# edouardlp/Mask-RCNN-CoreML

Hardware: AMD Instinct MI355X
Metric: images/sec (1024x1024, COCO-80) (higher is better)
Workload: dtype f32x3

## Files before the change

### mask-rcnn-coreml_amd/csrc/conv_dispatch.hip

```cpp
#include "conv_device.h"
#include "knobs.h"

namespace mrcnn {

void conv_mfma_launch(hipStream_t s, const ConvArgs& a, int mode, int bn, bool wide_waves);
void conv_pp_launch(hipStream_t s, const ConvArgs& a, int mode);
void conv_chain_launch(hipStream_t s, const ConvArgs& p, const ConvArgs& q, int parts, int n_cus, const void* p_stream, const void* q_stream);

static inline int conv_wdtype(const ConvDesc& d) { return d.wdtype < 0 ? d.dtype : d.wdtype; }
static inline bool conv_is_split(const ConvDesc& d) { return d.dtype == MRCNN_F32 && (conv_wdtype(d) == MRCNN_F16 || conv_wdtype(d) == MRCNN_F32X3); }
static inline int conv_split_parts(const ConvDesc& d) { return conv_wdtype(d) == MRCNN_F32X3 ? 3 : 2; }
static inline bool conv_is_f16(const ConvDesc& d) { return d.dtype == MRCNN_F16 && (d.wdtype < 0 || d.wdtype == MRCNN_F16) && !d.out_f32; }
static inline bool is_pointwise(const ConvDesc& d) { return d.KH == 1 && d.KW == 1 && d.stride == 1 && !d.padH && !d.padW; }
static inline bool is_3x3_same(const ConvDesc& d) { return d.KH == 3 && d.KW == 3 && d.stride == 1 && d.padH == 1 && d.padW == 1; }
static inline bool dense_in(const ConvDesc& d, int h, int w, int c) { return d.H == h && d.W == w && d.Cin == c && d.in_sW == c && d.in_sH == (long)w * c && d.in_sB == (long)h * w * c; }
static inline bool dense_out(const ConvDesc& d, int h, int w, int c) { return d.OH == h && d.OW == w && d.Cout == c && d.out_sP == c && d.out_sB == (long)h * w * c; }
static inline bool plain_epilogue(const ConvDesc& d, int act) { return !d.out2 && !d.deconv2 && !d.sel_partial && !d.head_w && d.res_shift == 0 && d.act == act && d.scale && d.shift; }
static inline bool fills_chip(long tiles, int n_cus) { return tiles * 8 >= (long)n_cus * 7; }

static thread_local ConvProfile* g_prof = nullptr;
void conv_set_profiler(ConvProfile* p) { g_prof = p; }
static thread_local int* g_range_flag = nullptr;
void conv_set_range_flag(int* device_flag) { g_range_flag = device_flag; }
void ConvProfile::reset()
// ... 43 lines not shown
}
static int prof_event(ConvProfile* p, hipStream_t s)
{
    if (p->used == (int)p->pool.size()) {
        hipEvent_t e;
        HIP_CHECK(hipEventCreate(&e));
        p->pool.push_back(e);
    }
    HIP_CHECK(hipEventRecord(p->pool[p->used], s));
    return p->used++;
}
struct ProfScope {
    ConvProfile* const prof = (g_prof && g_prof->active) ? g_prof : nullptr;
    const hipStream_t s;
    const int e0;
    explicit ProfScope(hipStream_t s_) : s(s_), e0(prof ? prof_event(prof, s_) : 0) {}
    explicit operator bool() const { return prof != nullptr; }
    void finish(ConvTileClass tile, double flops, int M, int N, int K, int group, double bytes) const
    {
        const int e1 = prof_event(prof, s);
        prof->pending.push_back({tile, flops, e0, e1, {M, N, K, tile}, group, bytes});
    }
};

int conv_n_tile(int Cout)
{
    if (Cout > 64) return 128;
    if (Cout > 32) return 64;
    return 32;
}

static int& g_min_blocks = knob("conv_min_blocks", nullptr, 448);
static int& g_min_blocks_split = knob("conv_min_blocks_split", nullptr, 256, "conv_min_blocks");
static inline int min_blocks_for(bool split_mode) { return split_mode ? g_min_blocks_split : g_min_blocks; }
static int& g_direct = knob("conv_direct", "MRCNN_DIRECT", 3);
static int& g_stem = knob("conv_stem", "MRCNN_STEM", 1);
static int& g_tail_dbg = knob("conv_tail_dbg", "MRCNN_TAIL_DBG", 0);
static int& g_tail = knob("conv_tail", "MRCNN_TAIL", 0);
static int& g_bneck = knob("conv_bneck", "MRCNN_BNECK", 1);
static int& g_bneck_stage = knob("conv_bneck_stage", "MRCNN_BNECK_STAGE", 0);
static int& g_c3h = knob("conv_c3h", "MRCNN_C3H", 1);
int conv_c3h_mode() { return g_c3h; }
bool conv_bneck_enabled() { return g_bneck != 0; }
static int& g_scfuse = knob("conv_scfuse", "MRCNN_SCFUSE", 1);
static int& g_sel_wave = knob("mask_sel_wave", "MRCNN_SEL_WAVE", 1);
int conv_sel_part_cols() { return g_sel_wave ? 64 : 128; }
static int& g_kchunk = knob("conv_kchunk", "MRCNN_KCHUNK", 1);
static int& g_ksplit = knob("conv_ksplit", "MRCNN_KSPLIT", 1);
static int& g_ksplit_below = knob("conv_ksplit_below", "MRCNN_KSPLIT_BELOW", 256);
static int& g_halo = knob("conv_halo", "MRCNN_HALO", 1);
bool conv_halo_enabled() { return g_halo != 0; }
static int& g_chain = knob("conv_chain", "MRCNN_CHAIN", 1);
static int& g_chain4 = knob("conv_chain4", "MRCNN_CHAIN4", 1);
static int& g_tn4 = knob("conv_tn4", nullptr, -1);

static int& g_pp = knob("conv_pp", "MRCNN_PP", 1);
static int& g_pp_min_tiles = knob("conv_pp_min_tiles", "MRCNN_PP_MIN_TILES", 512);
static int& g_pp_min_kt = knob("conv_pp_min_kt", "MRCNN_PP_MIN_KT", 16);
static int& g_pp_dbg = knob("conv_pp_dbg", "MRCNN_PP_DBG", 0);
static int& g_pp_min_fill = knob("conv_pp_min_fill", "MRCNN_PP_MIN_FILL", 85);
static int& g_pp_split = knob("conv_pp_split", "MRCNN_PP_SPLIT", 0);

static void conv_fill_args(const ConvDesc& d, ConvArgs& a)
{
    const bool half = d.dtype == MRCNN_F16;
    a.in = d.in; a.wgt = d.wgt; a.scale = d.scale; a.shift = d.shift; a.res = d.res; a.out = d.out; a.out2 = d.out2;
    a.in_sB = d.in_sB; a.in_sH = d.in_sH; a.in_sW = d.in_sW;
    a.res_sB = d.res_sB; a.res_sH = d.res_sH; a.res_sW = d.res_sW;
    a.out_sB = d.out_sB; a.out_sP = d.out_sP; a.out_sH = d.out_sH; a.out_sW = d.out_sW;
    a.out2_sB = d.out2_sB; a.out2_sP = d.out2_sP;
    a.B = d.B; a.H = d.H; a.W = d.W; a.Cin = d.Cin; a.KH = d.KH; a.KW = d.KW; a.stride = d.stride; a.padH = d.padH; a.padW = d.padW;
    a.OH = d.OH; a.OW = d.OW; a.Cout = d.Cout;
    a.ncols = d.deconv2 ? 4 * d.Cout : d.Cout;
    a.Ktot = d.KH * d.KW * d.Cin;
    const long M = (long)d.B * d.OH * d.OW;
    MRCNN_REQUIRE(M > 0 && M < (1L << 31) - 256, MRCNN_ERR_SHAPE, "conv: M out of range");
    a.M = (int)M;
    a.res_shift = d.res_shift; a.act = d.act; a.n_split = d.n_split; a.deconv2 = d.deconv2;
    a.out_f32 = (!half || d.out_f32) ? 1 : 0;
    a.range_flag = g_range_flag;
    a.dbg = g_pp_dbg;
    a.sel_w = d.sel_w; a.sel_cid = d.sel_cid; a.sel_partial = d.sel_partial;
    a.kchunks = 1; a.ksplit = 1; a.ks_scratch = nullptr; a.ks_count = nullptr;
    a.sel_part_cols = 128;
    a.sc_in = nullptr; a.sc_wgt = nullptr; a.sc_scale = nullptr; a.sc_shift = nullptr;
    a.sc_in_sB = a.sc_in_sH = a.sc_in_sW = 0; a.sc_H = a.sc_W = a.sc_Cin = 0; a.sc_stride = 1;
}

int conv_k_chunks(const ConvDesc& d)
{
    if (!g_kchunk || !conv_is_split(d) || d.KH != 1 || d.KW != 1 || d.Cin < 2048 || d.Cin % 32 != 0 || d.head_w) return 1;
    int n = d.Cin >= 8192 ? 8 : 4;
    while ((d.Cin / 32) % n) n >>= 1;
    return n;
}

static constexpr size_t KS_BYTES = 64u << 20;
static constexpr int KS_TILES = 8192;
static thread_local ConvScratch* g_scratch = nullptr;
void conv_set_scratch(ConvScratch* c) { g_scratch = c; }
size_t ConvScratch::ks_bytes() { return KS_BYTES; }
void ConvScratch::alloc()
{
    ks_buf.alloc(KS_BYTES);
    ks_cnt.alloc(KS_TILES * sizeof(unsigned));
    HIP_CHECK(hipMemset(ks_cnt.p, 0, KS_TILES * sizeof(unsigned)));
// ... 122 lines not shown
    if (pp_bn) conv_pp_launch(s, a, half ? 0 : parts);
    else conv_mfma_launch(s, a, half ? 0 : (split ? parts : 1), bn, wide_waves);
    if (prof) {
        const double k = (d.algo_k > 0 ? d.algo_k : a.Ktot) + (fuse ? sc->Cin : 0);
        const ConvTileClass tile = halo ? TILE_HALO : pp_bn == 256 ? TILE_PP_256x256 : (wide_waves ? TILE_128x128_4WAVE : (bn == 128 ? TILE_128x128 : (bn == 64 ? TILE_128x64 : TILE_128x32)));
        prof.finish(tile, 2.0 * (double)a.M * (double)a.ncols * k, a.M, a.ncols, a.Ktot, d.group, conv_algorithmic_bytes(d, fuse ? sc : nullptr));
    }
    HIP_CHECK(hipGetLastError());
}

bool conv_stem_enabled() { return g_stem != 0; }
bool conv_stem_eligible(const ConvDesc& d)
{
    const bool half = conv_is_f16(d);
    const int pxc = half ? 8 : 4;
    return (conv_is_split(d) || half) && d.KH == 7 && d.KW == 1 && d.Cin == 8 * pxc && d.stride == 2 && d.padH == 0 && d.padW == 0 && d.Cout == 64 && d.Npad == 64 &&
           d.act == ACT_RELU && !d.res && !d.out2 && !d.deconv2 && d.in_sW == pxc && d.in_sH == (long)d.W * pxc && d.in_sB == (long)d.H * d.W * pxc &&
           d.OH == (d.H - 7) / 2 + 1 && d.OW == (d.W - 7) / 2 + 1;
}

void conv_stem_forward(hipStream_t s, const ConvDesc& d, void* pooled, int PH, int PW)
{
    MRCNN_REQUIRE(conv_stem_eligible(d) && pooled && PH == (d.OH + 1) / 2 && PW == (d.OW + 1) / 2, MRCNN_ERR_INVALID, "conv_stem_forward: not the stem layer");
    const int n_cus = device_cu_count();
    const ProfScope prof(s);
    conv_stem_launch(s, d.in, d.B, d.H, d.W, d.wgt, d.scale, d.shift, d.OH, d.OW, pooled, PH, PW,
                     d.dtype == MRCNN_F16 ? 1 : conv_split_parts(d), g_range_flag, n_cus, g_stem != 2);
    if (prof) {
        const long M = (long)d.B * d.OH * d.OW;
        const double k = d.algo_k > 0 ? d.algo_k : d.KH * d.KW * d.Cin;
        const double by = (double)d.B * d.H * d.W * 16.0 + 64.0 * k * 2.0 + (double)d.B * PH * PW * 64.0 * (d.dtype == MRCNN_F16 ? 2.0 : 4.0);
        prof.finish(TILE_128x64, 2.0 * (double)M * 64.0 * k, (int)M, 64, d.KH * d.KW * d.Cin, d.group, by);
    }
}

bool conv_tail_fusable(const ConvDesc& d3, const ConvDesc& d1)
{
    if (!conv_is_split(d3) || !conv_is_split(d1) || conv_wdtype(d3) != conv_wdtype(d1)) return false;
    if (!d3.wgt_halo || !d1.wgt_halo || !conv_halo_eligible(d3) || d3.head_w || !conv_halo_tail_geometry_ok(d3.H, d3.W)) return false;
    if (d3.Npad != 256 || d3.act != ACT_RELU) return false;
    if (!conv_halo_tail_packable(d1.KH, d1.KW, d1.Cin, d1.Npad) || d1.Cout != 1024 || !is_pointwise(d1)) return false;
    if (d1.deconv2 || d1.out2 || d1.sel_partial || d1.act == ACT_SIGMOID || d1.res_shift || d1.head_w) return false;
    if (d1.in != d3.out || d1.B != d3.B || d1.OH != d3.OH || d1.OW != d3.OW) return false;
    if (!dense_out(d3, d3.OH, d3.OW, 256) || !dense_in(d1, d3.OH, d3.OW, 256)) return false;
    return true;
}

bool conv_chain_fusable(const ConvDesc& dP, const ConvDesc& dQ, const ConvDesc* sc)
{
    if (!conv_is_split(dP) || !conv_is_split(dQ) || conv_wdtype(dP) != conv_wdtype(dQ)) return false;
    const int C = dQ.Cout, H = dP.OH, W = dP.OW;
    if (!(C == 64 || C == 128 || C == 256) || dQ.Npad != C || dP.Cin != C || dP.Cout != 4 * C || dP.Npad != 4 * C) return false;
    if (!is_pointwise(dP) || !is_pointwise(dQ) || dP.B != dQ.B) return false;
    if (!plain_epilogue(dP, ACT_RELU) || !plain_epilogue(dQ, ACT_RELU) || dQ.res) return false;
    if (!dense_in(dP, H, W, C) || !dense_out(dP, H, W, 4 * C) || dQ.in != dP.out || !dense_in(dQ, H, W, 4 * C) || !dense_out(dQ, H, W, C)) return false;
    if (conv_k_chunks(dP) != 1 || conv_k_chunks(dQ) != 1) return false;
    auto al = [](const void* p) { return (reinterpret_cast<uintptr_t>(p) & 15) == 0; };
    if (!al(dP.in) || !al(dP.out) || !al(dQ.out) || !al(dP.wgt) || !al(dQ.wgt) || !al(dP.scale) || !al(dP.shift) || !al(dQ.scale) || !al(dQ.shift)) return false;
    if (C == 256 && (sc || !dP.wgt_stream || !dQ.wgt_stream || !al(dP.wgt_stream) || !al(dQ.wgt_stream))) return false;
    if (sc) {
        if (!g_scfuse || !conv_shortcut_fusable(dP, *sc) || conv_k_chunks(*sc) != 1 || !sc->scale || !sc->shift) return false;
        if (C == 64 && sc->Cin != 64) return false;
        if (!al(sc->in) || !al(sc->wgt) || !al(sc->scale) || !al(sc->shift) || sc->in_sW % 4 || sc->in_sH % 4 || sc->in_sB % 4 || sc->Npad != 4 * C) return false;
    } else {
        if (!dP.res || !al(dP.res) || dP.res_sW != 4 * C || dP.res_sH != (long)W * 4 * C || dP.res_sB != (long)H * W * 4 * C) return false;
    }
    return true;
}

void conv_forward_chain(hipStream_t s, const ConvDesc& dP, const ConvDesc& dQ, const ConvDesc* sc)
{
    const long tiles = ((long)dP.B * dP.OH * dP.OW + 127) / 128;
    const bool sc_rides = g_chain >= 3 ? sc != nullptr && conv_chain_fusable(dP, dQ, sc) : conv_shortcut_rides(dP, sc);
    const int n_cus = device_cu_count();
    const bool c4 = dQ.Cout == 256;
    const int g = c4 ? g_chain4 : g_chain;
    bool chain = g && g_direct >= 2 && !(c4 && sc) && conv_chain_fusable(dP, dQ, sc_rides ? sc : nullptr) && (g >= 2 || ((c4 || dQ.Cout == 64) && fills_chip(tiles, n_cus)));
#ifndef MRCNN_CONV_ABLATE
    if (g_pp_dbg) chain = false;
#endif
    if (!chain) {
        conv_forward(s, dP, sc);
        conv_forward(s, dQ);
        return;
    }
    if (sc && !sc_rides) { conv_forward(s, *sc); sc = nullptr; }
    ConvDesc d = dP;
    if (sc) { d.res = nullptr; d.res_sB = d.res_sH = d.res_sW = 0; }
    ConvArgs aP, aQ;
    conv_fill_args(d, aP);
    conv_fill_args(dQ, aQ);
    if (sc) {
        aP.sc_in = sc->in; aP.sc_wgt = sc->wgt; aP.sc_scale = sc->scale; aP.sc_shift = sc->shift;
        aP.sc_in_sB = sc->in_sB; aP.sc_in_sH = sc->in_sH; aP.sc_in_sW = sc->in_sW;
        aP.sc_H = sc->H; aP.sc_W = sc->W; aP.sc_Cin = sc->Cin; aP.sc_stride = sc->stride;
    }
    const ProfScope prof(s);
    conv_chain_launch(s, aP, aQ, conv_split_parts(dP), n_cus, dP.wgt_stream, dQ.wgt_stream);
    if (prof) {
        const double fl = 2.0 * (double)aP.M * ((double)aP.ncols * (aP.Ktot + (sc ? sc->Cin : 0)) + (double)aQ.ncols * aQ.Ktot);
        prof.finish(sc ? TILE_128x128_4WAVE : TILE_128x128, fl, aP.M, aP.ncols, aP.Ktot, dP.group,
                    conv_algorithmic_bytes(d, sc) + conv_algorithmic_bytes(dQ) - (double)aP.M * dQ.Cin * 4.0);
    }
    HIP_CHECK(hipGetLastError());
}

void conv_forward_tail(hipStream_t s, const ConvDesc& d3, const ConvDesc& d1, const ConvDesc* sc, const ConvDesc* q)
{
    const int n_cus = device_cu_count();
    const long tiles = ((long)d3.B * d3.OH * d3.OW + 127) / 128;
    ConvArgs a3, a1;
    bool fuse = g_tail && g_halo && g_scratch && conv_tail_fusable(d3, d1) && fills_chip(tiles, n_cus);
    if (sc && fuse) { conv_forward(s, *sc); sc = nullptr; }
    if (fuse) {
        conv_fill_args(d3, a3);
        conv_fill_args(d1, a1);
        a3.vec_ok = conv_vec_ok(d3, a3);
        a1.vec_ok = conv_vec_ok(d1, a1);
        a3.tiles_m = a1.tiles_m = 0; a3.tiles_n = a1.tiles_n = 0; a3.direct = a1.direct = 1;
        a1.dbg = g_tail_dbg;
        fuse = a3.vec_ok && a1.vec_ok && a3.dbg == 0;
    }
    if (!fuse) {
        conv_forward(s, d3);
        if (q) conv_forward_chain(s, d1, *q, sc);
        else conv_forward(s, d1, sc);
        return;
    }
    const ProfScope prof(s);
    (void)conv_halo_forward(s, a3, d3, conv_split_parts(d3), n_cus, &a1, d1.wgt_halo);
    if (prof) {
        const double fl = 2.0 * (double)a3.M * ((double)a3.ncols * a3.Ktot + (double)a1.ncols * a1.Ktot);
        ConvDesc d3n = d3; d3n.sel_partial = (float*)1;
        prof.finish(TILE_HALO_TAIL, fl, a3.M, a1.ncols, a3.Ktot + a1.Ktot, d3.group, conv_algorithmic_bytes(d3n) + conv_algorithmic_bytes(d1) - (double)a3.M * d1.Cin * 4.0);
    }
    HIP_CHECK(hipGetLastError());
    if (q) conv_forward(s, *q);
}

bool conv_bneck_fusable(const ConvDesc& da, const ConvDesc& db, const ConvDesc& dc)
{
    if (!conv_is_f16(da) || !conv_is_f16(db) || !conv_is_f16(dc)) return false;
    const int C = da.Cout, H = da.H, W = da.W;
    if (!(C == 64 || C == 128 || C == 256) || !bneck_geometry_ok(C, H, W)) return false;
    if (!plain_epilogue(da, ACT_RELU) || !plain_epilogue(db, ACT_RELU) || !plain_epilogue(dc, ACT_RELU) || da.res || db.res) return false;
    if (!is_pointwise(da) || !dense_in(da, H, W, 4 * C) || !dense_out(da, H, W, C)) return false;
    if (!is_3x3_same(db) || db.in != da.out || !dense_in(db, H, W, C) || !dense_out(db, H, W, C)) return false;
    if (!is_pointwise(dc) || dc.in != db.out || !dense_in(dc, H, W, C) || !dense_out(dc, H, W, 4 * C)) return false;
    if (dc.res != da.in || dc.res_sW != 4 * C || dc.res_sH != (long)W * 4 * C || dc.res_sB != (long)H * W * 4 * C) return false;
    if (dc.out == da.in) return false;
    if (da.B != db.B || da.B != dc.B) return false;
// ... 88 lines not shown
```

### mask-rcnn-coreml_amd/csrc/conv_pack.h

```cpp
#pragma once
#include <stddef.h>
#include <vector>

namespace mrcnn {

template <class Src>
std::vector<float> pack_filter_rows(int O, int I, int KH, int KW, int Npad, Src&& src)
{
    std::vector<float> w((size_t)Npad * KH * KW * I, 0.f);
    for (int o = 0; o < O; ++o)
        for (int y = 0; y < KH; ++y)
            for (int x = 0; x < KW; ++x)
                for (int i = 0; i < I; ++i) w[(((size_t)o * KH + y) * KW + x) * I + i] = src(o, y, x, i);
    return w;
}

inline int deconv2_row(int dy, int dx, int co, int O) { return (dy * 2 + dx) * O + co; }
template <class Src>
std::vector<float> pack_deconv2_rows(int I, int O, int Npad, Src&& src)
{
    std::vector<float> w((size_t)Npad * I, 0.f);
    for (int dy = 0; dy < 2; ++dy)
        for (int dx = 0; dx < 2; ++dx)
            for (int o = 0; o < O; ++o)
                for (int i = 0; i < I; ++i) w[(size_t)deconv2_row(dy, dx, o, O) * I + i] = src(dy, dx, o, i);
    return w;
}

inline bool chain_stream_wanted(int KH, int KW, int I, int O) { return KH == 1 && KW == 1 && ((I == 256 && O == 1024) || (I == 1024 && O == 256)); }
inline size_t chain_stream_pos_p(int C, int n, int k)
{
    const int r = n & 63;
    return (size_t)(n >> 6) * 64 * C + ((size_t)(k >> 5) * 64 + r) * 32 + ((((k >> 3) & 3) ^ ((r >> 2) & 3)) << 3) + (k & 7);
}
inline size_t chain_stream_pos_q(int C, int n, int k)
{
    return (size_t)(k >> 6) * 64 * C + ((size_t)((k >> 5) & 1) * C + n) * 32 + ((((k >> 3) & 3) ^ ((n >> 2) & 3)) << 3) + (k & 7);
}
template <class T>
std::vector<T> pack_chain_stream(const T* w, int C, bool q)
{
    static_assert(sizeof(T) == 2, "fp16 filters");
    const int rows = q ? C : 4 * C, K = q ? 4 * C : C;
    std::vector<T> img((size_t)rows * K);
    for (int n = 0; n < rows; ++n)
        for (int k = 0; k < K; ++k) img[q ? chain_stream_pos_q(C, n, k) : chain_stream_pos_p(C, n, k)] = w[(size_t)n * K + k];
    return img;
}

}
```

### mask-rcnn-coreml_amd/csrc/engine_weights.hip

```cpp
#include "engine_internal.h"
#include "conv_pack.h"

#include <math.h>
#include <string.h>

#include <fstream>

namespace mrcnn {

float half_to_float(uint16_t h)
{
    const uint32_t sign = (uint32_t)(h & 0x8000u) << 16;
    uint32_t exp = (h >> 10) & 0x1Fu, man = h & 0x3FFu, f;
    if (exp == 0) {
        if (man == 0) f = sign;
        else {
            exp = 113;
            while ((man & 0x400u) == 0) { man <<= 1; --exp; }
            man &= 0x3FFu;
            f = sign | (exp << 23) | (man << 13);
        }
    } else if (exp == 31) f = sign | 0x7F800000u | (man << 13);
    else f = sign | ((exp + 112) << 23) | (man << 13);
    float r;
// ... 146 lines not shown
    shift.assign(Npad, 0.f);
    if (bn.empty()) {
        for (int o = 0; o < Cout; ++o) { scale[o] = 1.f; shift[o] = bias[o]; }
        return;
    }
    const std::vector<float> g = f.floats(bn + "/gamma"), be = f.floats(bn + "/beta"), mu = f.floats(bn + "/mean"),
                             var = f.floats(bn + "/variance");
    const float eps = (float)f.get_double("bn_eps", 1e-3);
    for (int o = 0; o < Cout; ++o) {
        const float sc = g[o] / sqrtf(var[o] + eps);
        scale[o] = sc;
        shift[o] = (bias[o] - mu[o]) * sc + be[o];
    }
}

static PackedConv new_pack(int mode, int Cin, int Cout, int KH, int KW)
{
    PackedConv pc;
    pc.dtype = mode_act(mode); pc.wdtype = mode_wgt(mode);
    pc.Cin = Cin; pc.Cout = Cout; pc.KH = KH; pc.KW = KW;
    const int bn_tile = conv_n_tile(Cout);
    pc.Npad = (Cout + bn_tile - 1) / bn_tile * bn_tile;
    return pc;
}
static void finish_pack(PackedConv& pc, const std::vector<float>& w, const std::vector<float>& sc, const std::vector<float>& sh)
{
    upload_w(pc.wgt, w, pc.wdtype, pc.wdtype != pc.dtype, "MRCNN_F32S / MRCNN_F32X3");
    upload(pc.scale, sc);
    upload(pc.shift, sh);
    pc.h_scale = sc; pc.h_shift = sh;
}

PackedConv pack_conv_oihw(const MrcwFile& f, const std::string& conv, const std::string& bn, int dtype)
{
    const MrcwTensor& t = f.tensor(conv + "/kernel");
    MRCNN_REQUIRE(t.dims.size() == 4, MRCNN_ERR_IO, "%s/kernel is not 4-D", conv.c_str());
    const int O = t.dims[0], I = t.dims[1], KH = t.dims[2], KW = t.dims[3];
    const std::vector<float> k = f.floats(conv + "/kernel");
    PackedConv pc = new_pack(dtype, I, O, KH, KW);
    const std::vector<float> w = pack_filter_rows(O, I, KH, KW, pc.Npad, [&](int o, int y, int x, int i) { return k[(((size_t)o * I + i) * KH + y) * KW + x]; });
    std::vector<float> sc, sh;
    fold_bn(f, conv, bn, O, pc.Npad, sc, sh);
    finish_pack(pc, w, sc, sh);
    if (pc.wdtype != pc.dtype && conv_halo_packable(KH, KW, I, pc.Npad)) {
        conv_halo_pack(nullptr, pc.wgt.p, pc.Npad, I, pc.wgt_halo);
        HIP_CHECK(hipStreamSynchronize(nullptr));
    } else if (pc.wdtype != pc.dtype && conv_halo_tail_packable(KH, KW, I, pc.Npad) && O == pc.Npad) {
        conv_halo_pack(nullptr, pc.wgt.p, pc.Npad, I, pc.wgt_halo, 1);
        HIP_CHECK(hipStreamSynchronize(nullptr));
    }
    if (pc.wdtype != pc.dtype && pc.dtype == MRCNN_F32 && O == pc.Npad && chain_stream_wanted(KH, KW, I, O) && conv.find("_branch2") != std::string::npos) {
        std::vector<uint16_t> hw(w.size());
        for (size_t i = 0; i < w.size(); ++i) hw[i] = float_to_half(w[i]);
        const std::vector<uint16_t> img = pack_chain_stream(hw.data(), 256, I == 1024);
        pc.wgt_stream.alloc(img.size() * 2);
        HIP_CHECK(hipMemcpy(pc.wgt_stream.p, img.data(), img.size() * 2, hipMemcpyHostToDevice));
    }
    if (pc.dtype == MRCNN_F16 && pc.wdtype == MRCNN_F16 && conv3x3h_packable(KH, KW, I, O, pc.Npad)) {
        conv3x3h_pack(nullptr, pc.wgt.p, O, I, pc.wgt_c3h);
        HIP_CHECK(hipStreamSynchronize(nullptr));
    }
    if (pc.dtype == MRCNN_F16 && pc.wdtype == MRCNN_F16 && O == pc.Npad && bneck_frag_wanted(KH, KW, I, O)) {
        bneck_pack_frag(nullptr, pc.wgt.p, O, KH * KW * I, pc.wgt_frag);
        HIP_CHECK(hipStreamSynchronize(nullptr));
    }
    return pc;
}

PackedConv pack_conv1(const MrcwFile& f, int dtype)
{
    const MrcwTensor& t = f.tensor("conv1/kernel");
    MRCNN_REQUIRE(t.dims.size() == 4 && t.dims[1] == 3 && t.dims[2] == 7 && t.dims[3] == 7, MRCNN_ERR_IO, "conv1/kernel must be [O,3,7,7]");
    const int O = t.dims[0];
    const std::vector<float> k = f.floats("conv1/kernel");
    const int px = mode_act(dtype) == MRCNN_F16 ? 8 : 4;
    const int row = 8 * px;
    PackedConv pc = new_pack(dtype, row, O, 7, 1);
    std::vector<float> w((size_t)pc.Npad * 7 * row, 0.f);
    for (int o = 0; o < O; ++o)
        for (int ci = 0; ci < 3; ++ci)
            for (int y = 0; y < 7; ++y)
                for (int x = 0; x < 7; ++x)
                    w[((size_t)o * 7 + y) * row + x * px + ci] = k[(((size_t)o * 3 + ci) * 7 + y) * 7 + x];
    std::vector<float> sc, sh;
    fold_bn(f, "conv1", "bn_conv1", O, pc.Npad, sc, sh);
    finish_pack(pc, w, sc, sh);
    return pc;
}

PackedConv pack_stacked_1x1(const MrcwFile& f, const std::vector<std::string>& names, int dtype)
{
    int O = 0, I = -1;
    for (auto& n : names) {
        const MrcwTensor& t = f.tensor(n + "/kernel");
        MRCNN_REQUIRE(t.dims.size() == 2 || (t.dims.size() == 4 && t.dims[2] == 1 && t.dims[3] == 1), MRCNN_ERR_IO,
                      "%s/kernel is not an inner product / 1x1 kernel", n.c_str());
        MRCNN_REQUIRE(I < 0 || I == (int)t.dims[1], MRCNN_ERR_IO, "%s: input size mismatch", n.c_str());
        I = t.dims[1];
        O += t.dims[0];
    }
    PackedConv pc = new_pack(dtype, I, O, 1, 1);
    std::vector<float> w((size_t)pc.Npad * I, 0.f), sc(pc.Npad, 0.f), sh(pc.Npad, 0.f);
    int o0 = 0;
    for (auto& n : names) {
        const std::vector<float> k = f.floats(n + "/kernel"), b = f.floats(n + "/bias");
        memcpy(w.data() + (size_t)o0 * I, k.data(), k.size() * 4);
        for (size_t o = 0; o < b.size(); ++o) { sc[o0 + o] = 1.f; sh[o0 + o] = b[o]; }
// ... 33 lines not shown
```

### mask-rcnn-coreml_amd/csrc/kernels_conv_chain.hip

```cpp
#include "conv_device.h"

namespace mrcnn {

struct ChainArgs { ConvArgs p, q; const void *p_stream, *q_stream; };

__device__ __forceinline__ float4 chain_scale_shift(float4 x, const float4 sc, const float4 sh)
{
    x.x = x.x * sc.x + sh.x; x.y = x.y * sc.y + sh.y; x.z = x.z * sc.z + sh.z; x.w = x.w * sc.w + sh.w;
    return x;
}
__device__ __forceinline__ float4 chain_add(float4 x, const float4 r) { x.x += r.x; x.y += r.y; x.z += r.z; x.w += r.w; return x; }
__device__ __forceinline__ float4 chain_relu(float4 x) { x.x = fmaxf(x.x, 0.f); x.y = fmaxf(x.y, 0.f); x.z = fmaxf(x.z, 0.f); x.w = fmaxf(x.w, 0.f); return x; }
__device__ __forceinline__ bool chain_beyond_fp16(const float4 x) { return !(fabsf(x.x) < 65504.0f) || !(fabsf(x.y) < 65504.0f) || !(fabsf(x.z) < 65504.0f) || !(fabsf(x.w) < 65504.0f); }
__device__ __forceinline__ float4 chain_ld4(const float* p) { return *reinterpret_cast<const float4*>(p); }

struct ChainRows { bool ok[4]; long mrow[4]; int c4; };
__device__ __forceinline__ ChainRows chain_rows(int row0, int M, int lane)
{
    ChainRows rw;
    rw.c4 = (lane & 7) * 4;
#pragma unroll
    for (int ps = 0; ps < 4; ++ps) { const int m = row0 + 8 * ps + (lane >> 3); rw.ok[ps] = m < M; rw.mrow[ps] = m; }
    return rw;
}
// ... 256 lines not shown
            const int n = nc + j * 32 + rw.c4;
            if constexpr (SC) {
                tl.put(accS[j]);
                __builtin_amdgcn_wave_barrier();
                const float4 sc2 = chain_ld4(a.sc_scale + n), sh2 = chain_ld4(a.sc_shift + n);
#pragma unroll
                for (int ps = 0; ps < 4; ++ps) {
                    rv[j][ps] = chain_scale_shift(tl.row_get(ps), sc2, sh2);
                    out_of_range = out_of_range || chain_beyond_fp16(rv[j][ps]);
                }
                __builtin_amdgcn_wave_barrier();
            }
            tl.put(accP[j]);
            __builtin_amdgcn_wave_barrier();
            const float4 sc = chain_ld4(a.scale + n), sh = chain_ld4(a.shift + n);
            float4 xs[4];
#pragma unroll
            for (int ps = 0; ps < 4; ++ps) {
                float4 x = chain_scale_shift(tl.row_get(ps), sc, sh);
                if (SC || res) x = chain_add(x, rv[j][ps]);
                if (relu) x = chain_relu(x);
                if (rw.ok[ps]) {
                    out_of_range = out_of_range || chain_beyond_fp16(x);
                    *reinterpret_cast<float4*>(out + rw.mrow[ps] * C4 + n) = x;
                }
                xs[ps] = x;
            }
            __builtin_amdgcn_wave_barrier();
#pragma unroll
            for (int ps = 0; ps < 4; ++ps) tl.row_put(ps, xs[ps]);
            __builtin_amdgcn_wave_barrier();
#pragma unroll
            for (int g = 0; g < 2; ++g) {
                uint4 bq[TNQ];
#pragma unroll
                for (int jq = 0; jq < TNQ; ++jq) {
                    if constexpr (WLDS) bq[jq] = *reinterpret_cast<const uint4*>(smem + W_BYTES + ((nc / 32 + j) * C + jq * 32 + l31) * 64 + (((2 * g + kk) ^ swzb) << 4));
                    else bq[jq] = *reinterpret_cast<const uint4*>(w1 + (long)(jq * 32 + l31) * C4 + nc + j * 32 + g * 16 + 8 * kk);
                }
                chain_mfma_parts<PARTS, TNQ>(accQ, bq, tl.template frag<PARTS>(g));
            }
            __builtin_amdgcn_wave_barrier();
        }
    }
    chain_epilogue_q(tl, accQ, aq.scale, aq.shift, aq.act == ACT_RELU, rw, static_cast<float*>(aq.out), out_of_range_q);
    }
    if (a.range_flag && out_of_range) atomicOr(a.range_flag, 1);
    if (aq.range_flag && out_of_range_q) atomicOr(aq.range_flag, 1);
}

template <int C, int PARTS>
__global__ __launch_bounds__(512, 1) void k_conv_chain_ring(const ChainArgs ca)
{
    static_assert(C == 256, "the ring's stages hold C = 256's chunk images");
    constexpr int C4 = 4 * C, KT = C / 32, TNP = 2, TNQ = C / 32, NCH = C4 / 64, NPC = 2 * NCH;
    constexpr int WCH = 64 * C * 2;
    constexpr int WHALF = WCH / 2;
    constexpr int NW1 = 3;
    constexpr int W1_OFF = 2 * WCH, TILE_OFF = W1_OFF + NW1 * WHALF;
    __shared__ __attribute__((aligned(16))) unsigned char smem[TILE_OFF + 4 * 2 * 32 * 32 * 4];
    __shared__ __attribute__((aligned(16))) float s_tab[2 * C4], s_tabq[2 * C];
    const ConvArgs& a = ca.p;
    const ConvArgs& aq = ca.q;
    const int wave = __builtin_amdgcn_readfirstlane((int)threadIdx.x >> 6), lane = threadIdx.x & 63;
    const int pair = wave & 3;
    const int l31 = lane & 31, kk = lane >> 5;
    float* const tiles = reinterpret_cast<float*>(smem + TILE_OFF) + pair * (2 * 32 * 32);
    const ChainTile tx{tiles, lane}, ty{tiles + 32 * 32, lane};
    const int swzb = (l31 >> 2) & 3;
    const int row0 = (blockIdx.x * 4 + pair) * 32;
    const bool live = row0 < a.M;

    if (wave < 4) {
        const int t = pair * 64 + lane;
        static_assert(C4 == 4 * 256 && C % 8 == 0 && C / 2 <= 256, "the tables are filled by 256 threads, 16 B each");
        *reinterpret_cast<float4*>(&s_tab[4 * t]) = chain_ld4(a.scale + 4 * t);
        *reinterpret_cast<float4*>(&s_tab[C4 + 4 * t]) = chain_ld4(a.shift + 4 * t);
        if (t < C / 2) *reinterpret_cast<float4*>(&s_tabq[4 * t]) = chain_ld4(t < C / 4 ? aq.scale + 4 * t : aq.shift + 4 * (t - C / 4));
        typedef unsigned srd_t __attribute__((ext_vector_type(4)));
        srd_t srdP, srdQ;
        {
            const unsigned long long wp = (unsigned long long)(uintptr_t)ca.p_stream, wq = (unsigned long long)(uintptr_t)ca.q_stream;
            srdP[0] = __builtin_amdgcn_readfirstlane((unsigned)wp);
            srdP[1] = __builtin_amdgcn_readfirstlane((unsigned)(wp >> 32) & 0xffffu);
            srdP[2] = (unsigned)(NCH * WCH);
            srdP[3] = 0x00020000u;
            srdQ[0] = __builtin_amdgcn_readfirstlane((unsigned)wq);
            srdQ[1] = __builtin_amdgcn_readfirstlane((unsigned)(wq >> 32) & 0xffffu);
            srdQ[2] = (unsigned)(NCH * WCH);
            srdQ[3] = 0x00020000u;
        }
        const unsigned lds0 = __builtin_amdgcn_readfirstlane((unsigned)(uintptr_t)(__attribute__((address_space(3))) unsigned char*)smem);
        const unsigned wdst = lds0 + (unsigned)pair * 1024u;
        const unsigned voff = (unsigned)t * 16u;
#define MRCNN_RING_DMA(SRD, SOFF, DST)                                                                         \
    asm volatile("s_nop 4\n\ts_mov_b32 m0, %3\n\ts_nop 0\n\tbuffer_load_dwordx4 %0, %1, %2 offen lds" ::"v"(voff), "s"(SRD), "s"(SOFF), "s"(DST) : "memory", "m0");
        auto fill_w3 = [&](int c, int h) {
            const unsigned src = (unsigned)__builtin_amdgcn_readfirstlane(c) * (unsigned)WCH + (unsigned)(h * WHALF);
            const unsigned dst = wdst + (unsigned)(__builtin_amdgcn_readfirstlane(c) & 1) * (unsigned)WCH + (unsigned)(h * WHALF);
#pragma unroll
            for (int k = 0; k < WHALF / 4096; ++k) MRCNN_RING_DMA(srdP, src + k * 4096u, dst + k * 4096u)
        };
        auto fill_w1 = [&](int p) {
            const unsigned off = (unsigned)(__builtin_amdgcn_readfirstlane(p) & 1) * (unsigned)WHALF;
            const unsigned src = (unsigned)(__builtin_amdgcn_readfirstlane(p) >> 1) * (unsigned)WCH + off;
            const unsigned dst = wdst + (unsigned)W1_OFF + ((unsigned)__builtin_amdgcn_readfirstlane(p) % (unsigned)NW1) * (unsigned)WHALF;
#pragma unroll
            for (int k = 0; k < WHALF / 4096; ++k) MRCNN_RING_DMA(srdQ, src + k * 4096u, dst + k * 4096u)
        };
        fill_w3(0, 0);
        fill_w3(0, 1);
        auto ring_step = [&](int c, int h) {
            if (c + 1 < NCH) fill_w3(c + 1, h);
            fill_w1(2 * c + h);
        };
        uint4 u[2 * KT][2];
        {
            const int m = row0 + l31;
            const float* const src = static_cast<const float*>(a.in) + (long)m * C + 8 * kk;
#pragma unroll
            for (int g = 0; g < 2 * KT; ++g) {
                u[g][0] = u[g][1] = make_uint4(0u, 0u, 0u, 0u);
                if (m < a.M) { u[g][0] = *reinterpret_cast<const uint4*>(src + g * 16); u[g][1] = *reinterpret_cast<const uint4*>(src + g * 16 + 4); }
            }
        }
        f32x16 accP[TNP];
        chain_zero(accP);
        for (int c = 0; c < NCH; ++c) {
            const unsigned char* const w3s = smem + (c & 1) * WCH;
            auto frag_p = [&](uint4 (&b)[TNP], int i) {
#pragma unroll
                for (int j = 0; j < TNP; ++j) b[j] = *reinterpret_cast<const uint4*>(w3s + ((i >> 1) * 64 + j * 32 + l31) * 64 + (((2 * (i & 1) + kk) ^ swzb) << 4));
            };
#pragma unroll
            for (int h = 0; h < 2; ++h) {
                if (2 * c + h == 0 || c + 1 >= NCH) asm volatile("s_waitcnt vmcnt(0)" ::: "memory");
                else asm volatile("s_waitcnt vmcnt(8)" ::: "memory");
                __syncthreads();
                if (!live) { ring_step(c, h); continue; }
                if (h == 0) {
                    if (c > 0) ty.put(accP[1]);
                    chain_zero(accP);
                }
                uint4 bv[TNP];
                frag_p(bv, 8 * h);
                ChainParts pt = chain_split<PARTS>(u[8 * h][0], u[8 * h][1]);
#pragma unroll
                for (int i = 8 * h; i < 8 * h + 8; ++i) {
                    uint4 bn[TNP];
                    ChainParts pn;
                    if (i + 1 < 8 * h + 8) { frag_p(bn, i + 1); pn = chain_split<PARTS>(u[i + 1][0], u[i + 1][1]); }
                    chain_mfma_parts<PARTS, TNP>(accP, bv, pt);
                    if (i + 1 < 8 * h + 8) {
#pragma unroll
                        for (int j = 0; j < TNP; ++j) bv[j] = bn[j];
                        pt = pn;
                    }
                }
                ring_step(c, h);
                if (h == 1) tx.put(accP[0]);
            }
        }
        asm volatile("s_waitcnt vmcnt(0)" ::: "memory");
        __syncthreads();
        if (live) ty.put(accP[1]);
        asm volatile("s_waitcnt vmcnt(0)" ::: "memory");
        __syncthreads();
#undef MRCNN_RING_DMA
        return;
    }

    if (!live) {
        for (int s = 0; s < NPC + 2; ++s) __syncthreads();
        return;
    }
    const float* const res = static_cast<const float*>(a.res);
    float* const out = static_cast<float*>(a.out);
    const bool full = row0 + 32 <= a.M;
    const ChainRowOffs ro = chain_row_offs(row0, a.M, lane, C4);
    const float* const res0 = res + (long)row0 * C4;
    float* const out0 = out + (long)row0 * C4;
    const int c4 = (lane & 7) * 4;
    const bool relu = a.act == ACT_RELU;
    bool out_of_range = false, out_of_range_q = false;
    f32x16 accQ[TNQ];
    chain_zero(accQ);
    float4 rv[2][4];
    auto residual = [&](float4 (&r)[4], int p) { chain_residual_piece(r, res0 + p * 32, ro); };
    residual(rv[0], 0);
    __syncthreads();
    __syncthreads();
    for (int c = 0; c < NCH; ++c) {
#pragma unroll
        for (int j = 0; j < 2; ++j) {
            const int p = 2 * c + j;
            residual(rv[j ^ 1], p + 1 < NPC ? p + 1 : p);
            __syncthreads();
            const ChainTile& tl = j ? ty : tx;
            const unsigned char* const w1s = smem + W1_OFF + ((unsigned)p % (unsigned)NW1) * WHALF;
            auto frag_q = [&](uint4 (&b)[TNQ / 4], int h) {
#pragma unroll
                for (int i = 0; i < TNQ / 4; ++i) b[i] = *reinterpret_cast<const uint4*>(w1s + (((h & 3) * (TNQ / 4) + i) * 32 + l31) * 64 + (((2 * (h >> 2) + kk) ^ swzb) << 4));
            };
            uint4 bq[TNQ / 4];
            frag_q(bq, 0);
            const int n = p * 32 + c4;
            if (full) {
                if (relu) chain_piece_p<true, true>(tl, s_tab, s_tab + C4, rv[j], ro, out0 + p * 32, n, out_of_range);
                else chain_piece_p<true, false>(tl, s_tab, s_tab + C4, rv[j], ro, out0 + p * 32, n, out_of_range);
            } else {
                if (relu) chain_piece_p<false, true>(tl, s_tab, s_tab + C4, rv[j], ro, out0 + p * 32, n, out_of_range);
                else chain_piece_p<false, false>(tl, s_tab, s_tab + C4, rv[j], ro, out0 + p * 32, n, out_of_range);
            }
            ChainParts pt;
#pragma unroll
            for (int h = 0; h < 8; ++h) {
                if ((h & 3) == 0) pt = tl.template frag<PARTS>(h >> 2);
                uint4 bn[TNQ / 4];
                if (h < 7) frag_q(bn, h + 1);
                __builtin_amdgcn_sched_barrier(0);
                if ((h & 3) == 0) chain_mfma_parts<PARTS, TNQ / 4, TNQ, 0>(accQ, bq, pt);
                else if ((h & 3) == 1) chain_mfma_parts<PARTS, TNQ / 4, TNQ, TNQ / 4>(accQ, bq, pt);
                else if ((h & 3) == 2) chain_mfma_parts<PARTS, TNQ / 4, TNQ, TNQ / 2>(accQ, bq, pt);
                else chain_mfma_parts<PARTS, TNQ / 4, TNQ, 3 * TNQ / 4>(accQ, bq, pt);
                if (h < 7) {
#pragma unroll
                    for (int i = 0; i < TNQ / 4; ++i) bq[i] = bn[i];
                }
            }
            __builtin_amdgcn_wave_barrier();
        }
    }
    int lane_q = lane;
    asm volatile("" : "+v"(lane_q));
    chain_epilogue_q(tx, accQ, s_tabq, s_tabq + C, aq.act == ACT_RELU, chain_rows(row0, a.M, lane_q), static_cast<float*>(aq.out), out_of_range_q);
    if (a.range_flag && out_of_range) atomicOr(a.range_flag, 1);
    if (aq.range_flag && out_of_range_q) atomicOr(aq.range_flag, 1);
}


typedef void (*chain_kernel_t)(const ChainArgs);
template <int PARTS>
static chain_kernel_t chain_kernel(int C, bool sc)
{
    if (C == 256) return k_conv_chain_ring<256, PARTS>;
    if (C == 64) return sc ? k_conv_chain<64, PARTS, true> : k_conv_chain<64, PARTS, false>;
    return sc ? k_conv_chain<128, PARTS, true> : k_conv_chain<128, PARTS, false>;
}

void conv_chain_launch(hipStream_t s, const ConvArgs& p, const ConvArgs& q, int parts, int n_cus, const void* p_stream, const void* q_stream)
{
    ChainArgs ca{p, q, p_stream, q_stream};
    const bool sc = p.sc_in != nullptr;
    const int C = q.Cout;
    dim3 grid((p.M + 127) / 128), block(C == 256 ? 512 : 256);
    MRCNN_REQUIRE((C == 64 || C == 128 || C == 256) && (parts == 2 || parts == 3), MRCNN_ERR_INVALID, "conv_chain_launch: C %d, %d parts", C, parts);
    if (C == 256) MRCNN_REQUIRE(!sc && p.res && p_stream && q_stream, MRCNN_ERR_INVALID, "conv_chain_launch: C = 256 runs identity pairs from their stream images");
    if (C == 64) {
        MRCNN_REQUIRE((!sc || p.sc_Cin == 64) && n_cus > 0, MRCNN_ERR_INVALID, "conv_chain_launch: the LDS-resident form holds C = 64's filters");
        const int tiles256 = (p.M + 255) / 256;
        grid = dim3(tiles256 < n_cus ? tiles256 : n_cus); block = dim3(512);
    }
    hipLaunchKernelGGL(parts == 3 ? chain_kernel<3>(C, sc) : chain_kernel<2>(C, sc), grid, block, 0, s, ca);
}

}
```

Baseline: 477.9.

## Extend DMA-ring chain kernel to C=128 bottlenecks with persistent tile walking

Generalizes the streamed-weight ring chain kernel from C=256 to C=128 bottleneck pairs (1x1 expand then 1x1 reduce), packing stream weight images for 128/512 layers as well. For C=128 the kernel becomes persistent: grid is capped at the CU count and each block walks several tiles, prefetching the next tile's first weight chunk and residual while finishing the current one. The weight re-fetch and launch cost of per-tile blocks should shrink, and weight DMA overlaps with compute. In exchange the pair no longer carries a fused shortcut, the control flow and LDS ring indexing get more complex, and the dispatch also starts accepting a non-ReLU first stage.

```diff
diff --git a/mask-rcnn-coreml_amd/csrc/conv_dispatch.hip b/mask-rcnn-coreml_amd/csrc/conv_dispatch.hip
--- a/mask-rcnn-coreml_amd/csrc/conv_dispatch.hip
+++ b/mask-rcnn-coreml_amd/csrc/conv_dispatch.hip
@@ -119,6 +119,9 @@
 bool conv_halo_enabled() { return g_halo != 0; }
 static int& g_chain = knob("conv_chain", "MRCNN_CHAIN", 1);
 static int& g_chain4 = knob("conv_chain4", "MRCNN_CHAIN4", 1);
+static int& g_chain3 = knob("conv_chain3", "MRCNN_CHAIN3", 1);
+static int& g_chain3_entry = knob("conv_chain3_entry", "MRCNN_CHAIN3_ENTRY", 0);
+static int& g_chain3_grid = knob("conv_chain3_grid", "MRCNN_CHAIN3_GRID", 0);
 static int& g_tn4 = knob("conv_tn4", nullptr, -1);
 
 static int& g_pp = knob("conv_pp", "MRCNN_PP", 1);
@@ -347,12 +350,13 @@
     const int C = dQ.Cout, H = dP.OH, W = dP.OW;
     if (!(C == 64 || C == 128 || C == 256) || dQ.Npad != C || dP.Cin != C || dP.Cout != 4 * C || dP.Npad != 4 * C) return false;
     if (!is_pointwise(dP) || !is_pointwise(dQ) || dP.B != dQ.B) return false;
-    if (!plain_epilogue(dP, ACT_RELU) || !plain_epilogue(dQ, ACT_RELU) || dQ.res) return false;
+    if ((!plain_epilogue(dP, ACT_RELU) && !plain_epilogue(dP, ACT_NONE)) || !plain_epilogue(dQ, ACT_RELU) || dQ.res) return false;
     if (!dense_in(dP, H, W, C) || !dense_out(dP, H, W, 4 * C) || dQ.in != dP.out || !dense_in(dQ, H, W, 4 * C) || !dense_out(dQ, H, W, C)) return false;
     if (conv_k_chunks(dP) != 1 || conv_k_chunks(dQ) != 1) return false;
     auto al = [](const void* p) { return (reinterpret_cast<uintptr_t>(p) & 15) == 0; };
     if (!al(dP.in) || !al(dP.out) || !al(dQ.out) || !al(dP.wgt) || !al(dQ.wgt) || !al(dP.scale) || !al(dP.shift) || !al(dQ.scale) || !al(dQ.shift)) return false;
     if (C == 256 && (sc || !dP.wgt_stream || !dQ.wgt_stream || !al(dP.wgt_stream) || !al(dQ.wgt_stream))) return false;
+    if ((dP.wgt_stream && !al(dP.wgt_stream)) || (dQ.wgt_stream && !al(dQ.wgt_stream))) return false;
     if (sc) {
         if (!g_scfuse || !conv_shortcut_fusable(dP, *sc) || conv_k_chunks(*sc) != 1 || !sc->scale || !sc->shift) return false;
         if (C == 64 && sc->Cin != 64) return false;
@@ -366,11 +370,14 @@
 void conv_forward_chain(hipStream_t s, const ConvDesc& dP, const ConvDesc& dQ, const ConvDesc* sc)
 {
     const long tiles = ((long)dP.B * dP.OH * dP.OW + 127) / 128;
-    const bool sc_rides = g_chain >= 3 ? sc != nullptr && conv_chain_fusable(dP, dQ, sc) : conv_shortcut_rides(dP, sc);
+    const bool sc_rides_alone = g_chain >= 3 ? sc != nullptr && conv_chain_fusable(dP, dQ, sc) : conv_shortcut_rides(dP, sc);
     const int n_cus = device_cu_count();
     const bool c4 = dQ.Cout == 256;
+    const bool ring3 = dQ.Cout == 128 && g_chain3 && g_direct >= 2 && dP.wgt_stream && dQ.wgt_stream && (g_chain3 >= 2 || ((!sc || g_chain3_entry) && fills_chip(tiles, n_cus))) &&
+                       conv_chain_fusable(dP, dQ, nullptr);
+    const bool sc_rides = ring3 ? false : sc_rides_alone;
     const int g = c4 ? g_chain4 : g_chain;
-    bool chain = g && g_direct >= 2 && !(c4 && sc) && conv_chain_fusable(dP, dQ, sc_rides ? sc : nullptr) && (g >= 2 || ((c4 || dQ.Cout == 64) && fills_chip(tiles, n_cus)));
+    bool chain = ring3 || (g && g_direct >= 2 && !(c4 && sc) && conv_chain_fusable(dP, dQ, sc_rides ? sc : nullptr) && (g >= 2 || ((c4 || dQ.Cout == 64) && fills_chip(tiles, n_cus))));
 #ifndef MRCNN_CONV_ABLATE
     if (g_pp_dbg) chain = false;
 #endif
@@ -391,7 +398,8 @@
         aP.sc_H = sc->H; aP.sc_W = sc->W; aP.sc_Cin = sc->Cin; aP.sc_stride = sc->stride;
     }
     const ProfScope prof(s);
-    conv_chain_launch(s, aP, aQ, conv_split_parts(dP), n_cus, dP.wgt_stream, dQ.wgt_stream);
+    const bool ring = c4 || ring3;
+    conv_chain_launch(s, aP, aQ, conv_split_parts(dP), ring3 && g_chain3_grid > 0 ? g_chain3_grid : n_cus, ring ? dP.wgt_stream : nullptr, ring ? dQ.wgt_stream : nullptr);
     if (prof) {
         const double fl = 2.0 * (double)aP.M * ((double)aP.ncols * (aP.Ktot + (sc ? sc->Cin : 0)) + (double)aQ.ncols * aQ.Ktot);
         prof.finish(sc ? TILE_128x128_4WAVE : TILE_128x128, fl, aP.M, aP.ncols, aP.Ktot, dP.group,
diff --git a/mask-rcnn-coreml_amd/csrc/conv_pack.h b/mask-rcnn-coreml_amd/csrc/conv_pack.h
--- a/mask-rcnn-coreml_amd/csrc/conv_pack.h
+++ b/mask-rcnn-coreml_amd/csrc/conv_pack.h
@@ -27,7 +27,12 @@
     return w;
 }
 
-inline bool chain_stream_wanted(int KH, int KW, int I, int O) { return KH == 1 && KW == 1 && ((I == 256 && O == 1024) || (I == 1024 && O == 256)); }
+inline int chain_stream_c(int I, int O) { return I < O ? I : O; }
+inline bool chain_stream_wanted(int KH, int KW, int I, int O)
+{
+    const int C = chain_stream_c(I, O);
+    return KH == 1 && KW == 1 && (C == 256 || C == 128) && (I == 4 * C || O == 4 * C);
+}
 inline size_t chain_stream_pos_p(int C, int n, int k)
 {
     const int r = n & 63;
diff --git a/mask-rcnn-coreml_amd/csrc/engine_weights.hip b/mask-rcnn-coreml_amd/csrc/engine_weights.hip
--- a/mask-rcnn-coreml_amd/csrc/engine_weights.hip
+++ b/mask-rcnn-coreml_amd/csrc/engine_weights.hip
@@ -222,7 +222,7 @@
     if (pc.wdtype != pc.dtype && pc.dtype == MRCNN_F32 && O == pc.Npad && chain_stream_wanted(KH, KW, I, O) && conv.find("_branch2") != std::string::npos) {
         std::vector<uint16_t> hw(w.size());
         for (size_t i = 0; i < w.size(); ++i) hw[i] = float_to_half(w[i]);
-        const std::vector<uint16_t> img = pack_chain_stream(hw.data(), 256, I == 1024);
+        const std::vector<uint16_t> img = pack_chain_stream(hw.data(), chain_stream_c(I, O), I > O);
         pc.wgt_stream.alloc(img.size() * 2);
         HIP_CHECK(hipMemcpy(pc.wgt_stream.p, img.data(), img.size() * 2, hipMemcpyHostToDevice));
     }
diff --git a/mask-rcnn-coreml_amd/csrc/kernels_conv_chain.hip b/mask-rcnn-coreml_amd/csrc/kernels_conv_chain.hip
--- a/mask-rcnn-coreml_amd/csrc/kernels_conv_chain.hip
+++ b/mask-rcnn-coreml_amd/csrc/kernels_conv_chain.hip
@@ -332,12 +332,15 @@
 template <int C, int PARTS>
 __global__ __launch_bounds__(512, 1) void k_conv_chain_ring(const ChainArgs ca)
 {
-    static_assert(C == 256, "the ring's stages hold C = 256's chunk images");
+    static_assert(C == 256 || C == 128, "the ring's stages hold a chunk image of C = 256 or C = 128");
+    constexpr bool WALK = C == 128;
     constexpr int C4 = 4 * C, KT = C / 32, TNP = 2, TNQ = C / 32, NCH = C4 / 64, NPC = 2 * NCH;
+    constexpr int GH = KT;
     constexpr int WCH = 64 * C * 2;
     constexpr int WHALF = WCH / 2;
     constexpr int NW1 = 3;
     constexpr int W1_OFF = 2 * WCH, TILE_OFF = W1_OFF + NW1 * WHALF;
+    static_assert(WHALF % 4096 == 0 && NCH % 2 == 0 && TNQ % 4 == 0, "4 KB DMA rounds; W3's stage of chunk 0 is the same in every tile; Q's quarters");
     __shared__ __attribute__((aligned(16))) unsigned char smem[TILE_OFF + 4 * 2 * 32 * 32 * 4];
     __shared__ __attribute__((aligned(16))) float s_tab[2 * C4], s_tabq[2 * C];
     const ConvArgs& a = ca.p;
@@ -348,14 +351,18 @@
     float* const tiles = reinterpret_cast<float*>(smem + TILE_OFF) + pair * (2 * 32 * 32);
     const ChainTile tx{tiles, lane}, ty{tiles + 32 * 32, lane};
     const int swzb = (l31 >> 2) & 3;
-    const int row0 = (blockIdx.x * 4 + pair) * 32;
-    const bool live = row0 < a.M;
+    const int ntiles = (a.M + 127) >> 7;
+    int tile = blockIdx.x;
+    int row0 = (tile * 4 + pair) * 32;
+    bool live = row0 < a.M;
 
     if (wave < 4) {
         const int t = pair * 64 + lane;
-        static_assert(C4 == 4 * 256 && C % 8 == 0 && C / 2 <= 256, "the tables are filled by 256 threads, 16 B each");
-        *reinterpret_cast<float4*>(&s_tab[4 * t]) = chain_ld4(a.scale + 4 * t);
-        *reinterpret_cast<float4*>(&s_tab[C4 + 4 * t]) = chain_ld4(a.shift + 4 * t);
+        static_assert(C4 <= 4 * 256 && C % 8 == 0 && C / 2 <= 256, "the tables are filled by 256 threads, 16 B each");
+        if (C4 == 4 * 256 || t < C4 / 4) {
+            *reinterpret_cast<float4*>(&s_tab[4 * t]) = chain_ld4(a.scale + 4 * t);
+            *reinterpret_cast<float4*>(&s_tab[C4 + 4 * t]) = chain_ld4(a.shift + 4 * t);
+        }
         if (t < C / 2) *reinterpret_cast<float4*>(&s_tabq[4 * t]) = chain_ld4(t < C / 4 ? aq.scale + 4 * t : aq.shift + 4 * (t - C / 4));
         typedef unsigned srd_t __attribute__((ext_vector_type(4)));
         srd_t srdP, srdQ;
@@ -381,19 +388,26 @@
 #pragma unroll
             for (int k = 0; k < WHALF / 4096; ++k) MRCNN_RING_DMA(srdP, src + k * 4096u, dst + k * 4096u)
         };
-        auto fill_w1 = [&](int p) {
+        auto fill_w1 = [&](int p, int gp) {
             const unsigned off = (unsigned)(__builtin_amdgcn_readfirstlane(p) & 1) * (unsigned)WHALF;
             const unsigned src = (unsigned)(__builtin_amdgcn_readfirstlane(p) >> 1) * (unsigned)WCH + off;
-            const unsigned dst = wdst + (unsigned)W1_OFF + ((unsigned)__builtin_amdgcn_readfirstlane(p) % (unsigned)NW1) * (unsigned)WHALF;
+            const unsigned dst = wdst + (unsigned)W1_OFF + ((unsigned)__builtin_amdgcn_readfirstlane(gp) % (unsigned)NW1) * (unsigned)WHALF;
 #pragma unroll
             for (int k = 0; k < WHALF / 4096; ++k) MRCNN_RING_DMA(srdQ, src + k * 4096u, dst + k * 4096u)
         };
         fill_w3(0, 0);
         fill_w3(0, 1);
+        int gp0 = 0;
+        bool more = WALK && tile + (int)gridDim.x < ntiles;
         auto ring_step = [&](int c, int h) {
             if (c + 1 < NCH) fill_w3(c + 1, h);
-            fill_w1(2 * c + h);
+            else if (more) fill_w3(0, h);
+            fill_w1(2 * c + h, gp0 + 2 * c + h);
         };
+        f32x16 accP[TNP];
+        chain_zero(accP);
+        bool owed = false;
+        for (;;) {
         uint4 u[2 * KT][2];
         {
             const int m = row0 + l31;
@@ -404,8 +418,6 @@
                 if (m < a.M) { u[g][0] = *reinterpret_cast<const uint4*>(src + g * 16); u[g][1] = *reinterpret_cast<const uint4*>(src + g * 16 + 4); }
             }
         }
-        f32x16 accP[TNP];
-        chain_zero(accP);
         for (int c = 0; c < NCH; ++c) {
             const unsigned char* const w3s = smem + (c & 1) * WCH;
             auto frag_p = [&](uint4 (&b)[TNP], int i) {
@@ -414,52 +426,65 @@
             };
 #pragma unroll
             for (int h = 0; h < 2; ++h) {
-                if (2 * c + h == 0 || c + 1 >= NCH) asm volatile("s_waitcnt vmcnt(0)" ::: "memory");
-                else asm volatile("s_waitcnt vmcnt(8)" ::: "memory");
+                if (2 * c + h == 0 || (c + 1 >= NCH && !more)) asm volatile("s_waitcnt vmcnt(0)" ::: "memory");
+                else if constexpr (WHALF / 4096 == 4) asm volatile("s_waitcnt vmcnt(8)" ::: "memory");
+                else { static_assert(WHALF / 4096 == 4 || WHALF / 4096 == 2, "vmcnt(2 x WHALF / 4 KB)"); asm volatile("s_waitcnt vmcnt(4)" ::: "memory"); }
                 __syncthreads();
+                if constexpr (WALK) {
+                    if (h == 0 && owed) { ty.put(accP[1]); owed = false; }
+                }
                 if (!live) { ring_step(c, h); continue; }
                 if (h == 0) {
-                    if (c > 0) ty.put(accP[1]);
+                    if (!WALK && c > 0) ty.put(accP[1]);
                     chain_zero(accP);
                 }
                 uint4 bv[TNP];
-                frag_p(bv, 8 * h);
-                ChainParts pt = chain_split<PARTS>(u[8 * h][0], u[8 * h][1]);
-#pragma unroll
-                for (int i = 8 * h; i < 8 * h + 8; ++i) {
+                frag_p(bv, GH * h);
+                ChainParts pt = chain_split<PARTS>(u[GH * h][0], u[GH * h][1]);
+#pragma unroll
+                for (int i = GH * h; i < GH * h + GH; ++i) {
                     uint4 bn[TNP];
                     ChainParts pn;
-                    if (i + 1 < 8 * h + 8) { frag_p(bn, i + 1); pn = chain_split<PARTS>(u[i + 1][0], u[i + 1][1]); }
+                    if (i + 1 < GH * h + GH) { frag_p(bn, i + 1); pn = chain_split<PARTS>(u[i + 1][0], u[i + 1][1]); }
                     chain_mfma_parts<PARTS, TNP>(accP, bv, pt);
-                    if (i + 1 < 8 * h + 8) {
+                    if (i + 1 < GH * h + GH) {
 #pragma unroll
                         for (int j = 0; j < TNP; ++j) bv[j] = bn[j];
                         pt = pn;
                     }
                 }
                 ring_step(c, h);
-                if (h == 1) tx.put(accP[0]);
-            }
+                if (h == 1) { tx.put(accP[0]); owed = true; }
+            }
+        }
+        if (!more) break;
+        tile += gridDim.x;
+        gp0 += NPC;
+        row0 = (tile * 4 + pair) * 32;
+        live = row0 < a.M;
+        more = tile + (int)gridDim.x < ntiles;
         }
         asm volatile("s_waitcnt vmcnt(0)" ::: "memory");
         __syncthreads();
-        if (live) ty.put(accP[1]);
+        if (WALK ? owed : live) ty.put(accP[1]);
         asm volatile("s_waitcnt vmcnt(0)" ::: "memory");
         __syncthreads();
 #undef MRCNN_RING_DMA
         return;
     }
 
-    if (!live) {
-        for (int s = 0; s < NPC + 2; ++s) __syncthreads();
-        return;
+    if constexpr (!WALK) {
+        if (!live) {
+            for (int s = 0; s < NPC + 2; ++s) __syncthreads();
+            return;
+        }
     }
     const float* const res = static_cast<const float*>(a.res);
     float* const out = static_cast<float*>(a.out);
-    const bool full = row0 + 32 <= a.M;
-    const ChainRowOffs ro = chain_row_offs(row0, a.M, lane, C4);
-    const float* const res0 = res + (long)row0 * C4;
-    float* const out0 = out + (long)row0 * C4;
+    bool full = row0 + 32 <= a.M;
+    ChainRowOffs ro = chain_row_offs(row0, a.M, lane, C4);
+    const float* res0 = res + (long)row0 * C4;
+    float* out0 = out + (long)row0 * C4;
     const int c4 = (lane & 7) * 4;
     const bool relu = a.act == ACT_RELU;
     bool out_of_range = false, out_of_range_q = false;
@@ -467,17 +492,25 @@
     chain_zero(accQ);
     float4 rv[2][4];
     auto residual = [&](float4 (&r)[4], int p) { chain_residual_piece(r, res0 + p * 32, ro); };
-    residual(rv[0], 0);
+    if (!WALK || live) residual(rv[0], 0);
     __syncthreads();
     __syncthreads();
+    int gp0 = 0;
+    for (;;) {
+    const bool more = WALK && tile + (int)gridDim.x < ntiles;
     for (int c = 0; c < NCH; ++c) {
 #pragma unroll
         for (int j = 0; j < 2; ++j) {
             const int p = 2 * c + j;
-            residual(rv[j ^ 1], p + 1 < NPC ? p + 1 : p);
+            if (!WALK || live) {
+                const int rown = row0 + (int)gridDim.x * 128;
+                if (WALK && p + 1 == NPC && more && rown < a.M) chain_residual_piece(rv[0], res + (long)rown * C4, chain_row_offs(rown, a.M, lane, C4));
+                else residual(rv[j ^ 1], p + 1 < NPC ? p + 1 : p);
+            }
             __syncthreads();
+            if (WALK && !live) continue;
             const ChainTile& tl = j ? ty : tx;
-            const unsigned char* const w1s = smem + W1_OFF + ((unsigned)p % (unsigned)NW1) * WHALF;
+            const unsigned char* const w1s = smem + W1_OFF + ((unsigned)(gp0 + p) % (unsigned)NW1) * WHALF;
             auto frag_q = [&](uint4 (&b)[TNQ / 4], int h) {
 #pragma unroll
                 for (int i = 0; i < TNQ / 4; ++i) b[i] = *reinterpret_cast<const uint4*>(w1s + (((h & 3) * (TNQ / 4) + i) * 32 + l31) * 64 + (((2 * (h >> 2) + kk) ^ swzb) << 4));
@@ -511,9 +544,22 @@
             __builtin_amdgcn_wave_barrier();
         }
     }
-    int lane_q = lane;
-    asm volatile("" : "+v"(lane_q));
-    chain_epilogue_q(tx, accQ, s_tabq, s_tabq + C, aq.act == ACT_RELU, chain_rows(row0, a.M, lane_q), static_cast<float*>(aq.out), out_of_range_q);
+    if (!WALK || live) {
+        int lane_q = lane;
+        asm volatile("" : "+v"(lane_q));
+        chain_epilogue_q(WALK ? ty : tx, accQ, s_tabq, s_tabq + C, aq.act == ACT_RELU, chain_rows(row0, a.M, lane_q), static_cast<float*>(aq.out), out_of_range_q);
+    }
+    if (!more) break;
+    chain_zero(accQ);
+    tile += gridDim.x;
+    gp0 += NPC;
+    row0 = (tile * 4 + pair) * 32;
+    live = row0 < a.M;
+    full = row0 + 32 <= a.M;
+    ro = chain_row_offs(row0, a.M, lane, C4);
+    res0 = res + (long)row0 * C4;
+    out0 = out + (long)row0 * C4;
+    }
     if (a.range_flag && out_of_range) atomicOr(a.range_flag, 1);
     if (aq.range_flag && out_of_range_q) atomicOr(aq.range_flag, 1);
 }
@@ -521,9 +567,10 @@
 
 typedef void (*chain_kernel_t)(const ChainArgs);
 template <int PARTS>
-static chain_kernel_t chain_kernel(int C, bool sc)
+static chain_kernel_t chain_kernel(int C, bool sc, bool ring)
 {
     if (C == 256) return k_conv_chain_ring<256, PARTS>;
+    if (C == 128 && ring) return k_conv_chain_ring<128, PARTS>;
     if (C == 64) return sc ? k_conv_chain<64, PARTS, true> : k_conv_chain<64, PARTS, false>;
     return sc ? k_conv_chain<128, PARTS, true> : k_conv_chain<128, PARTS, false>;
 }
@@ -533,15 +580,20 @@
     ChainArgs ca{p, q, p_stream, q_stream};
     const bool sc = p.sc_in != nullptr;
     const int C = q.Cout;
-    dim3 grid((p.M + 127) / 128), block(C == 256 ? 512 : 256);
+    const bool ring = C == 256 || (C == 128 && p_stream && q_stream);
+    dim3 grid((p.M + 127) / 128), block(ring ? 512 : 256);
     MRCNN_REQUIRE((C == 64 || C == 128 || C == 256) && (parts == 2 || parts == 3), MRCNN_ERR_INVALID, "conv_chain_launch: C %d, %d parts", C, parts);
-    if (C == 256) MRCNN_REQUIRE(!sc && p.res && p_stream && q_stream, MRCNN_ERR_INVALID, "conv_chain_launch: C = 256 runs identity pairs from their stream images");
+    if (ring) MRCNN_REQUIRE(!sc && p.res && p_stream && q_stream, MRCNN_ERR_INVALID, "conv_chain_launch: the ring form runs pairs with a residual tensor from their stream images");
+    if (ring && C == 128) {
+        MRCNN_REQUIRE(n_cus > 0, MRCNN_ERR_INVALID, "conv_chain_launch: the walking ring's grid");
+        if ((int)grid.x > n_cus) grid = dim3(n_cus);
+    }
     if (C == 64) {
         MRCNN_REQUIRE((!sc || p.sc_Cin == 64) && n_cus > 0, MRCNN_ERR_INVALID, "conv_chain_launch: the LDS-resident form holds C = 64's filters");
         const int tiles256 = (p.M + 255) / 256;
         grid = dim3(tiles256 < n_cus ? tiles256 : n_cus); block = dim3(512);
     }
-    hipLaunchKernelGGL(parts == 3 ? chain_kernel<3>(C, sc) : chain_kernel<2>(C, sc), grid, block, 0, s, ca);
-}
-
-}
+    hipLaunchKernelGGL(parts == 3 ? chain_kernel<3>(C, sc, ring) : chain_kernel<2>(C, sc, ring), grid, block, 0, s, ca);
+}
+
+}
```

After: 481.4 (median of 6 runs). About the same (+0.7%).
